# PecanProject/sipnet

Measured on AMD Instinct MI355X. Metric: ensemble-site-timesteps/sec, higher is better.
Workload: dtype f64; 1 GPU; c10k: 1 site(s) x 10240 members per GPU x 17520 half-hourly steps, perturbed params, default flags; sites_per_gpu=1, fast_math=True, gather=n/a (1 GPU), parallelism=ensemble-sharded x1, ranks_seen=1, devices_seen=1, kernel=stepCoopKernel<double, true, true, false>

## Files before the change

sipnet_amd/_lib.py:

```python
import ctypes as C
import os

_HERE = os.path.dirname(os.path.abspath(__file__))
LIB_PATH = os.path.join(_HERE, "libsipnet_amd.so")

NPARAMS, NFLAGS, NCLIM, NREC, NSTATE, RING_SLOTS = 80, 12, 11, 44, 32, 250
NDBG = 72
NREC_OUT = 36

OK = 0
ERR_BAD_PARAMETER = 3
ERR_UNKNOWN_EVENT = 4
ERR_INPUT_FILE = 5
ERR_FILE_OPEN = 6
ERR_INTERNAL = 7
ERR_BAD_CLI = 8
ERR_RESTART = 9
ERR_NO_DEVICE = 100
ERR_BAD_ARGUMENT = 101

F64, F32_MIXED = 0, 1
KERNEL_AUTO, KERNEL_ONE_WAVE, KERNEL_COOP_LDS, KERNEL_COOP_HBM, KERNEL_STRICT, KERNEL_COOP_PAIR, KERNEL_COOP_QUAD = range(7)
KERNEL_COOP_NCYCLE = 7
KERNEL_COOP_NCYCLE_PAIR = 8
# ... 170 lines not shown
    "sipnet_node_pf_check": (C.c_int, [_P, _I32P]),
    "sipnet_node_pf_ancestors": (_P, [_P, C.c_int32]),
    "sipnet_node_pf_block_len": (C.c_int64, [_P]),
    "sipnet_node_destroy": (None, [_P]),
    "sipnet_node_n_devices": (C.c_int32, [_P]),
    "sipnet_node_batch": (_P, [_P, C.c_int32]),
    "sipnet_node_run_gathering_reduced": (C.c_int, [_P, C.c_int32, C.c_int32, C.c_int32, C.c_int32, C.c_int32]),
    "sipnet_node_gathered_reduced": (_P, [_P, C.c_int32, C.c_int32, _P, _P, _P]),
    "sipnet_node_reduced_in_kernel": (C.c_int32, [_P]),
    "sipnet_node_member_range": (C.c_int, [_P, C.c_int32, _I32P, _I32P]),
    "sipnet_node_collective_library": (C.c_char_p, [_P]),
    "sipnet_comm_unique_id": (C.c_int, [_P]),
    "sipnet_comm_create": (C.c_int, [_P, C.c_int32, C.c_int32, C.c_int32, C.POINTER(_P)]),
    "sipnet_comm_all_gather": (C.c_int, [_P, _P, _P, C.c_int64, _P]),
    "sipnet_comm_world": (C.c_int32, [_P]),
    "sipnet_comm_destroy": (None, [_P]),
    "sipnet_node_set_climate": (C.c_int, [_P, C.c_int32, C.c_int32, _P, _P, _P]),
    "sipnet_node_set_events": (C.c_int, [_P, C.c_int32, C.c_int32, _P]),
    "sipnet_node_set_params": (C.c_int, [_P, C.c_int32, C.c_int32, C.c_int32, _P]),
    "sipnet_node_set_math": (C.c_int, [_P, C.c_int32]),
    "sipnet_node_set_kernel": (C.c_int, [_P, C.c_int32, C.c_int32]),
    "sipnet_node_setup": (C.c_int, [_P]),
    "sipnet_node_run": (C.c_int, [_P, C.c_int32, C.c_int32]),
    "sipnet_node_sync": (C.c_int, [_P]),
    "sipnet_node_ld": (C.c_int64, [_P]),
    "sipnet_node_planes": (_P, [_P, C.c_int32]),
    "sipnet_node_stats": (_P, [_P, C.c_int32]),
    "sipnet_node_gather_stats": (C.c_int, [_P, _P]),
    "sipnet_node_gathered_stats": (_P, [_P, C.c_int32]),
    "sipnet_node_gather_planes": (C.c_int, [_P]),
    "sipnet_node_gathered_planes": (_P, [_P, C.c_int32]),
    "sipnet_node_run_gathering": (C.c_int, [_P, C.c_int32, C.c_int32, C.c_int32]),
    "sipnet_node_n_segments": (C.c_int32, [_P]),
    "sipnet_node_gathered_segment": (_P, [_P, C.c_int32, C.c_int32, C.POINTER(C.c_int32), C.POINTER(C.c_int32)]),
    "sipnet_batch_ncol": (C.c_int64, [_P]),
    "sipnet_batch_nsteps": (C.c_int32, [_P]),
    "sipnet_batch_site_nsteps": (C.c_int32, [_P, C.c_int32]),
    "sipnet_batch_get_site_series": (C.c_int, [_P, C.c_int32, _P, _P]),
    "sipnet_batch_last_kernel_ms": (C.c_double, [_P]),
    "sipnet_batch_time_next_launch": (C.c_int, [_P]),
    "sipnet_batch_pf_arm": (C.c_int, [_P, C.c_double, C.c_double, _P]),
    "sipnet_dev_alloc": (_P, [C.c_size_t]),
    "sipnet_dev_free": (None, [_P]),
    "sipnet_dev_to_host": (C.c_int, [_P, _P, C.c_size_t, _P]),
    "sipnet_dev_to_host_2d": (C.c_int, [_P, C.c_size_t, _P, C.c_size_t, C.c_size_t, C.c_size_t, _P]),
    "sipnet_dev_to_dev_2d": (C.c_int, [_P, C.c_size_t, _P, C.c_size_t, C.c_size_t, C.c_size_t, _P]),
    "sipnet_batch_set_climate_sites": (C.c_int, [_P, C.c_int32, C.c_int32, _P, _P, _P, _P]),
    "sipnet_debug_plan_compare": (C.c_int, [_P, C.c_int32, C.c_int32, _P, _P, _P, _P, _P]),
    "sipnet_batch_run_sums": (C.c_int, [_P, C.c_int32, C.c_int32, C.c_int32, _P, _P, _P, C.c_int64, _P]),
    "sipnet_batch_sums_in_kernel": (C.c_int32, [_P]),
    "sipnet_debug_set_num_cus": (C.c_int, [_P, C.c_int32]),
    "sipnet_debug_pf_barrier": (C.c_int, [_P, C.c_int32, C.c_int32]),
    "sipnet_batch_set_device_share": (C.c_int, [_P, C.c_int32]),
    "sipnet_batch_pf_info": (C.c_int, [_P, _P, _P]),
    "sipnet_stream_sync": (C.c_int, [_P]),
    "sipnet_stream_create": (_P, [C.c_int32]),
    "sipnet_stream_destroy": (None, [_P]),
    "sipnet_io_read_clim": (C.c_int, [C.c_char_p, C.c_int32, C.POINTER(_P)]),
    "sipnet_clim_nsteps": (C.c_int32, [_P]),
    "sipnet_clim_data": (_DP, [_P]),
    "sipnet_clim_year": (_I32P, [_P]),
    "sipnet_clim_day": (_I32P, [_P]),
    "sipnet_clim_free": (None, [_P]),
    "sipnet_io_read_params": (C.c_int, [C.c_char_p, _I32P, _P, _P]),
    "sipnet_param_name": (C.c_char_p, [C.c_int32]),
    "sipnet_param_index": (C.c_int32, [C.c_char_p]),
    "sipnet_io_read_events": (C.c_int, [C.c_char_p, _I32P, _P, C.POINTER(C.POINTER(Event)), _I32P]),
    "sipnet_io_free": (None, [_P]),
    "sipnet_io_format_out_header": (C.c_int, [C.c_char_p, C.c_size_t]),
    "sipnet_io_format_out_row": (C.c_int, [C.c_char_p, C.c_size_t, C.c_int32, C.c_int32, C.c_double, _P, C.c_int64]),
    "sipnet_io_write_out": (C.c_int, [C.c_char_p, C.c_int32, C.c_int32, _P, _P, _P, _P]),
    "sipnet_io_write_debug_logs": (C.c_int, [C.c_char_p, C.c_int32, C.c_int32, _P, _P, _P, _P, _P]),
    "sipnet_io_write_events_out": (C.c_int, [C.c_char_p, C.c_int32, _I32P, _P, C.c_int32, _P, _P, _P,
                                             C.c_int32, _P, _P, _P]),
    "sipnet_io_ensemble_create": (C.c_int, [C.c_char_p, C.c_int32, C.c_int32, _P, _P, _P, _P, C.c_int32, _P, _P,
                                            C.c_int32, C.c_char_p, C.POINTER(_P)]),
    "sipnet_io_ensemble_put": (C.c_int, [_P, C.c_int32, C.c_int32, C.c_int32, C.c_int32, C.c_int32, _P, C.c_int64,
                                         C.c_int32]),
    "sipnet_io_ensemble_close": (C.c_int, [_P]),
    "sipnet_io_out_column_count": (C.c_int32, []),
    "sipnet_io_out_column_index": (C.c_int32, [C.c_char_p]),
    "sipnet_io_out_column": (C.c_int, [C.c_int32, C.POINTER(C.c_char_p), _I32P, _I32P, C.POINTER(C.c_char_p)]),
    "sipnet_io_write_ensemble_block": (C.c_int, [C.c_char_p, C.c_int32, C.c_int32, _P, _P, _P, _P, _P, _P, C.c_int64,
                                                 C.c_char_p, C.c_int32, C.c_char_p]),
    "sipnet_io_read_restart": (C.c_int, [C.c_char_p, _P]),
    "sipnet_io_write_restart": (C.c_int, [C.c_char_p, _P]),
    "sipnet_restart_check": (C.c_int, [_P, _I32P, C.c_int32, C.c_int32, C.c_int32, C.c_double,
                                       C.c_double, _I32P]),
    "sipnet_restart_check_boundary_for_write": (C.c_int, [_P, _I32P]),
}

_lib = None
_DEV_LIBRARY = False


def use_library(path):
    global LIB_PATH, _DEV_LIBRARY
    if _lib is not None:
        raise RuntimeError("sipnet_amd: the library is already loaded")
    LIB_PATH = os.path.abspath(path)
    _DEV_LIBRARY = True


def lib():
    global _lib
    if _lib is None:
        if not os.path.exists(LIB_PATH):
            raise ImportError(
                f"{LIB_PATH} is missing: the HIP extension has not been built. "
                "Run `python -c 'import __graft_entry__ as g; g.build()'`. "
                "sipnet_amd has no CPU fallback.")
        try:
            import torch
        except Exception:
            pass
        _lib = C.CDLL(LIB_PATH)
        for name, (res, args) in SIGNATURES.items():
            if _DEV_LIBRARY and not hasattr(_lib, name):
                continue
            fn = getattr(_lib, name)
            fn.restype = res
            fn.argtypes = args
    return _lib


def _strip_comments(text):
    out, i, n = [], 0, len(text)
    while i < n:
        c = text[i]
        if c in "\"'":
            j = i + 1
            while j < n and text[j] != c:
                j += 2 if text[j] == "\\" else 1
            out.append(text[i:j + 1])
            i = j + 1
        elif text.startswith("//", i):
            j = text.find("\n", i)
            i = n if j < 0 else j
        elif text.startswith("/*", i):
            j = text.find("*/", i + 2)
            i = n if j < 0 else j + 2
            out.append(" ")
        else:
            out.append(c)
            i += 1
    return " ".join("".join(out).split())


def kernel_source_sha16():
    import hashlib
    h = hashlib.sha256()
    csrc = os.path.join(_HERE, "csrc")
    for name in ("step_kernel.hip", "step_fast.hip", "fast_body.inc", "step_coop.hip", "coop_mailboxes.inc", "coop_stats.inc", "coop_wave_carbon.inc",
                 "coop_wave_factor.inc", "coop_wave_light.inc", "coop_wave_soil.inc", "coop_wave_water.inc", "step_kernel.h",
                 "fast_math.h", "coop_probes.h", "plan.h"):
        h.update(name.encode())
        h.update(_strip_comments(open(os.path.join(csrc, name), "r", errors="replace").read()).encode())
    return h.hexdigest()[:16]


class SipnetError(RuntimeError):
    def __init__(self, code, where=""):
        self.code = code
        msg = lib().sipnet_last_error().decode(errors="replace")
        super().__init__(f"{where}: status {code}: {msg}")


def check(code, where=""):
    if code != OK:
        raise SipnetError(code, where)
```

sipnet_amd/csrc/step_coop.hip:

```cpp
#include <hip/hip_runtime.h>

#include <cstdio>
#include <type_traits>

#include "fast_math.h"
#include "step_kernel.h"

namespace sipnet {
#ifdef SIPNET_COOP_BOUNDED
namespace bounded {
#endif
#ifdef SIPNET_COOP_SUMS_TU
namespace sums2 {
#endif
namespace {

constexpr int kTileBytes = kFastTile * (int)sizeof(FastRec);

#ifdef SIPNET_COOP_BOUNDED
__device__ unsigned long long g_coopStuck[2];
__shared__ int g_coopPoison;
constexpr int kSpinBudget = 1 << 22;
__device__ __forceinline__ bool spinOut(int& n, int id, int step) {
  n++;
  if ((n & 255) != 1) return false;
  int p;
  asm volatile("ds_read_b32 %0, %1\n\ts_waitcnt lgkmcnt(0)" : "=v"(p) : "v"((unsigned)(size_t)&g_coopPoison) : "memory");
  if (__builtin_amdgcn_readfirstlane(p)) return true;
  if (n < kSpinBudget) return false;
  if ((threadIdx.x & 63) == 0) {
    const unsigned long long rep = (1ull << 63) | ((unsigned long long)(unsigned)id << 32) | (unsigned)step;
    if (atomicCAS(&g_coopStuck[0], 0ull, rep) == 0ull) g_coopStuck[1] = blockIdx.x;
  }
  asm volatile("ds_write_b32 %0, %1" :: "v"((unsigned)(size_t)&g_coopPoison), "v"(1) : "memory");
  return true;
}
#define WAIT_DO for (int spin_ = 0, once_ = 1; once_; once_ = 0) do
#define WAIT_WHILE(cond, id, step) while ((cond) && !spinOut(spin_, id, step))
#else
#define WAIT_DO do
#define WAIT_WHILE(cond, id, step) while (cond)
#endif

__device__ __forceinline__ void post(double* slot, int* flag, double v, int step) {
  asm volatile("ds_write_b64 %0, %1\n\tds_write_b32 %2, %3"
               :: "v"((unsigned)(size_t)slot), "v"(v), "v"((unsigned)(size_t)flag), "v"(step) : "memory");
}
__device__ __forceinline__ void post(float* slot, int* flag, float v, int step) {
  asm volatile("ds_write_b32 %0, %1\n\tds_write_b32 %2, %3"
               :: "v"((unsigned)(size_t)slot), "v"(v), "v"((unsigned)(size_t)flag), "v"(step) : "memory");
}
__device__ __forceinline__ double take(const double* slot, const int* flag, int step) {
  double v;
  int f;
  WAIT_DO {
    asm volatile("ds_read_b32 %0, %2\n\tds_read_b64 %1, %3\n\ts_waitcnt lgkmcnt(0)"
                 : "=&v"(f), "=&v"(v) : "v"((unsigned)(size_t)flag), "v"((unsigned)(size_t)slot) : "memory");
  } WAIT_WHILE(uni(f) < step, 1, step);
  return v;
}
__device__ __forceinline__ float take(const float* slot, const int* flag, int step) {
  float v;
  int f;
  WAIT_DO {
    asm volatile("ds_read_b32 %0, %2\n\tds_read_b32 %1, %3\n\ts_waitcnt lgkmcnt(0)"
                 : "=&v"(f), "=&v"(v) : "v"((unsigned)(size_t)flag), "v"((unsigned)(size_t)slot) : "memory");
  } WAIT_WHILE(uni(f) < step, 2, step);
  return v;
}
typedef double d2_t __attribute__((ext_vector_type(2)));
typedef int i4_t __attribute__((ext_vector_type(4)));
__device__ __forceinline__ unsigned ldsAddr(const void* p) { return (unsigned)(size_t)p; }
template <class R>
__device__ __forceinline__ R q10Arg(R t10, R lg) {
  R x = t10 * lg;
  asm volatile("" : "+v"(x));
  return x;
}
__device__ __forceinline__ int aliveWord(int step, bool died) { return died ? -(step + 2) : (step + 2); }
__device__ __forceinline__ void postAlive(int* slot, int step, bool died) {
  asm volatile("ds_write_b32 %0, %1" :: "v"((unsigned)(size_t)slot), "v"(aliveWord(step, died)) : "memory");
}
__device__ __forceinline__ void takePgp(const double* slot, const int* flag, const int* alive, int step,
                                        double& pgp, bool& died) {
  int f, w;
  WAIT_DO {
    asm volatile("ds_read_b32 %0, %3\n\tds_read_b64 %1, %4\n\tds_read_b32 %2, %5\n\ts_waitcnt lgkmcnt(0)"
                 : "=&v"(f), "=&v"(pgp), "=&v"(w)
                 : "v"((unsigned)(size_t)flag), "v"((unsigned)(size_t)slot), "v"((unsigned)(size_t)alive) : "memory");
  } WAIT_WHILE(uni(f) < step || uni(w < 0 ? -w : w) < step + 2, 3, step);
  died = w < 0;
}
__device__ __forceinline__ void takePgp(const float* slot, const int* flag, const int* alive, int step,
                                        float& pgp, bool& died) {
  int f, w;
  WAIT_DO {
    asm volatile("ds_read_b32 %0, %3\n\tds_read_b32 %1, %4\n\tds_read_b32 %2, %5\n\ts_waitcnt lgkmcnt(0)"
                 : "=&v"(f), "=&v"(pgp), "=&v"(w)
                 : "v"((unsigned)(size_t)flag), "v"((unsigned)(size_t)slot), "v"((unsigned)(size_t)alive) : "memory");
  } WAIT_WHILE(uni(f) < step || uni(w < 0 ? -w : w) < step + 2, 4, step);
  died = w < 0;
}
typedef double d2v __attribute__((ext_vector_type(2)));
typedef float f2v __attribute__((ext_vector_type(2)));
typedef int i2v __attribute__((ext_vector_type(2)));
__device__ __forceinline__ void takeFactors(const double* block, const int* flags2, int step, double& g1,
                                            double& g2, double& qSoilT, double& gFine, double& gCoarse,
                                            double& moist) {
  i2v f;
  d2v a, b, c;
  WAIT_DO {
    asm volatile("ds_read2_b32 %0, %4 offset1:1\n\tds_read2st64_b64 %1, %5 offset1:1\n\t"
                 "ds_read2st64_b64 %2, %5 offset0:2 offset1:3\n\tds_read2st64_b64 %3, %5 offset0:4 offset1:5\n\t"
                 "s_waitcnt lgkmcnt(0)"
                 : "=&v"(f), "=&v"(a), "=&v"(b), "=&v"(c)
                 : "v"((unsigned)(size_t)flags2), "v"((unsigned)(size_t)block) : "memory");
  } WAIT_WHILE(uni(f.x < f.y ? f.x : f.y) < step, 5, step);
  g1 = a.x; g2 = a.y; qSoilT = b.x; gFine = b.y; gCoarse = c.x; moist = c.y;
}
__device__ __forceinline__ void takeFactors(const float* block, const int* flags2, int step, float& g1,
                                            float& g2, float& qSoilT, float& gFine, float& gCoarse, float& moist) {
  i2v f;
  f2v a, b, c;
  WAIT_DO {
    asm volatile("ds_read2_b32 %0, %4 offset1:1\n\tds_read2st64_b32 %1, %5 offset1:1\n\t"
                 "ds_read2st64_b32 %2, %5 offset0:2 offset1:3\n\tds_read2st64_b32 %3, %5 offset0:4 offset1:5\n\t"
                 "s_waitcnt lgkmcnt(0)"
                 : "=&v"(f), "=&v"(a), "=&v"(b), "=&v"(c)
                 : "v"((unsigned)(size_t)flags2), "v"((unsigned)(size_t)block) : "memory");
  } WAIT_WHILE(uni(f.x < f.y ? f.x : f.y) < step, 6, step);
  g1 = a.x; g2 = a.y; qSoilT = b.x; gFine = b.y; gCoarse = c.x; moist = c.y;
}
__device__ __forceinline__ void takeFactorsN(const double* block, const int* facFlag, const double* minNSlot, const int* minNFlag,
                                             int step, double& g1, double& g2, double& gFine, double& gCoarse, double& qSoil,
                                             double& minN, int& minNSeq) {
  int f0, f1;
  d2v a, b;
  WAIT_DO {
    asm volatile("ds_read_b32 %0, %6\n\tds_read2st64_b64 %1, %7 offset1:1\n\tds_read2st64_b64 %2, %7 offset0:3 offset1:4\n\t"
                 "ds_read_b64 %3, %7 offset:3072\n\tds_read_b32 %4, %8\n\tds_read_b64 %5, %9\n\ts_waitcnt lgkmcnt(0)"
                 : "=&v"(f0), "=&v"(a), "=&v"(b), "=&v"(qSoil), "=&v"(f1), "=&v"(minN)
                 : "v"((unsigned)(size_t)facFlag), "v"((unsigned)(size_t)block), "v"((unsigned)(size_t)minNFlag),
                   "v"((unsigned)(size_t)minNSlot) : "memory");
  } WAIT_WHILE(uni(f0) < step, 7, step);
  minNSeq = uni(f1);
  g1 = a.x; g2 = a.y; gFine = b.x; gCoarse = b.y;
}
__device__ __forceinline__ void takeFactorsN(const float* block, const int* facFlag, const double* minNSlot, const int* minNFlag,
                                             int step, float& g1, float& g2, float& gFine, float& gCoarse, float& qSoil,
                                             double& minN, int& minNSeq) {
  int f0, f1;
  f2v a, b;
  WAIT_DO {
    asm volatile("ds_read_b32 %0, %6\n\tds_read2st64_b32 %1, %7 offset1:1\n\tds_read2st64_b32 %2, %7 offset0:3 offset1:4\n\t"
                 "ds_read_b32 %3, %7 offset:1536\n\tds_read_b32 %4, %8\n\tds_read_b64 %5, %9\n\ts_waitcnt lgkmcnt(0)"
                 : "=&v"(f0), "=&v"(a), "=&v"(b), "=&v"(qSoil), "=&v"(f1), "=&v"(minN)
                 : "v"((unsigned)(size_t)facFlag), "v"((unsigned)(size_t)block), "v"((unsigned)(size_t)minNFlag),
                   "v"((unsigned)(size_t)minNSlot) : "memory");
  } WAIT_WHILE(uni(f0) < step, 8, step);
  minNSeq = uni(f1);
  g1 = a.x; g2 = a.y; gFine = b.x; gCoarse = b.y;
}
__device__ __forceinline__ void takeFactorsRing(const double* block, const int* flags2, unsigned ringAddr,
                                                int step, double& g1, double& g2, double& qSoilT,
                                                double& gFine, double& gCoarse, double& moist, double& ringV) {
  i2v f;
  d2v a, b, c;
  WAIT_DO {
    asm volatile("ds_read2_b32 %0, %5 offset1:1\n\tds_read2st64_b64 %1, %6 offset1:1\n\t"
                 "ds_read2st64_b64 %2, %6 offset0:2 offset1:3\n\tds_read2st64_b64 %3, %6 offset0:4 offset1:5\n\t"
                 "ds_read_b64 %4, %7\n\ts_waitcnt lgkmcnt(0)"
                 : "=&v"(f), "=&v"(a), "=&v"(b), "=&v"(c), "=&v"(ringV)
                 : "v"((unsigned)(size_t)flags2), "v"((unsigned)(size_t)block), "v"(ringAddr) : "memory");
  } WAIT_WHILE(uni(f.x < f.y ? f.x : f.y) < step, 9, step);
  g1 = a.x; g2 = a.y; qSoilT = b.x; gFine = b.y; gCoarse = c.x; moist = c.y;
}
__device__ __forceinline__ void takeFactorsRing(const float* block, const int* flags2, unsigned ringAddr,
                                                int step, float& g1, float& g2, float& qSoilT, float& gFine,
                                                float& gCoarse, float& moist, double& ringV) {
  i2v f;
  f2v a, b, c;
  WAIT_DO {
    asm volatile("ds_read2_b32 %0, %5 offset1:1\n\tds_read2st64_b32 %1, %6 offset1:1\n\t"
                 "ds_read2st64_b32 %2, %6 offset0:2 offset1:3\n\tds_read2st64_b32 %3, %6 offset0:4 offset1:5\n\t"
                 "ds_read_b64 %4, %7\n\ts_waitcnt lgkmcnt(0)"
                 : "=&v"(f), "=&v"(a), "=&v"(b), "=&v"(c), "=&v"(ringV)
                 : "v"((unsigned)(size_t)flags2), "v"((unsigned)(size_t)block), "v"(ringAddr) : "memory");
  } WAIT_WHILE(uni(f.x < f.y ? f.x : f.y) < step, 10, step);
  g1 = a.x; g2 = a.y; qSoilT = b.x; gFine = b.y; gCoarse = c.x; moist = c.y;
}
__device__ __forceinline__ void post5(double* base, int* flag, double v0, double v1, double v2, double v3,
                                      double v4, int step) {
  asm volatile("ds_write2st64_b64 %0, %1, %2 offset1:1\n\tds_write2st64_b64 %0, %3, %4 offset0:2 offset1:3\n\t"
               "ds_write_b64 %0, %5 offset:2048\n\tds_write_b32 %6, %7"
               :: "v"(ldsAddr(base)), "v"(v0), "v"(v1), "v"(v2), "v"(v3), "v"(v4), "v"(ldsAddr(flag)), "v"(step)
               : "memory");
}
__device__ __forceinline__ void post5(float* base, int* flag, float v0, float v1, float v2, float v3,
                                      float v4, int step) {
  asm volatile("ds_write2st64_b32 %0, %1, %2 offset1:1\n\tds_write2st64_b32 %0, %3, %4 offset0:2 offset1:3\n\t"
               "ds_write_b32 %0, %5 offset:1024\n\tds_write_b32 %6, %7"
               :: "v"(ldsAddr(base)), "v"(v0), "v"(v1), "v"(v2), "v"(v3), "v"(v4), "v"(ldsAddr(flag)), "v"(step)
               : "memory");
}
__device__ __forceinline__ void post2(double* base, int* flag, double v0, double v1, int step) {
  asm volatile("ds_write2st64_b64 %0, %1, %2 offset1:1\n\tds_write_b32 %3, %4"
               :: "v"(ldsAddr(base)), "v"(v0), "v"(v1), "v"(ldsAddr(flag)), "v"(step) : "memory");
}
__device__ __forceinline__ void post2(float* base, int* flag, float v0, float v1, int step) {
  asm volatile("ds_write2st64_b32 %0, %1, %2 offset1:1\n\tds_write_b32 %3, %4"
               :: "v"(ldsAddr(base)), "v"(v0), "v"(v1), "v"(ldsAddr(flag)), "v"(step) : "memory");
}
__device__ __forceinline__ void takeFactors7(const double* block, const int* flags2, int step, double& g1, double& g2,
                                             double& qSoilT, double& gFine, double& gCoarse, double& moist, double& mK) {
  i2v f;
  d2v a, b, c;
  WAIT_DO {
    asm volatile("ds_read2_b32 %0, %5 offset1:1\n\tds_read2st64_b64 %1, %6 offset1:1\n\t"
                 "ds_read2st64_b64 %2, %6 offset0:2 offset1:3\n\tds_read2st64_b64 %3, %6 offset0:4 offset1:5\n\t"
                 "ds_read_b64 %4, %6 offset:3072\n\ts_waitcnt lgkmcnt(0)"
                 : "=&v"(f), "=&v"(a), "=&v"(b), "=&v"(c), "=&v"(mK)
                 : "v"((unsigned)(size_t)flags2), "v"((unsigned)(size_t)block) : "memory");
  } WAIT_WHILE(uni(f.x < f.y ? f.x : f.y) < step, 11, step);
  g1 = a.x; g2 = a.y; qSoilT = b.x; gFine = b.y; gCoarse = c.x; moist = c.y;
}
__device__ __forceinline__ void takeFactors7(const float* block, const int* flags2, int step, float& g1, float& g2,
                                             float& qSoilT, float& gFine, float& gCoarse, float& moist, float& mK) {
  i2v f;
  f2v a, b, c;
  WAIT_DO {
    asm volatile("ds_read2_b32 %0, %5 offset1:1\n\tds_read2st64_b32 %1, %6 offset1:1\n\t"
                 "ds_read2st64_b32 %2, %6 offset0:2 offset1:3\n\tds_read2st64_b32 %3, %6 offset0:4 offset1:5\n\t"
                 "ds_read_b32 %4, %6 offset:1536\n\ts_waitcnt lgkmcnt(0)"
                 : "=&v"(f), "=&v"(a), "=&v"(b), "=&v"(c), "=&v"(mK)
                 : "v"((unsigned)(size_t)flags2), "v"((unsigned)(size_t)block) : "memory");
  } WAIT_WHILE(uni(f.x < f.y ? f.x : f.y) < step, 12, step);
  g1 = a.x; g2 = a.y; qSoilT = b.x; gFine = b.y; gCoarse = c.x; moist = c.y;
}
__device__ __forceinline__ void takeFactorsRing7(const double* block, const int* flags2, unsigned ringAddr, int step,
                                                 double& g1, double& g2, double& qSoilT, double& gFine, double& gCoarse,
                                                 double& moist, double& mK, double& ringV) {
  i2v f;
  d2v a, b, c;
  WAIT_DO {
    asm volatile("ds_read2_b32 %0, %6 offset1:1\n\tds_read2st64_b64 %1, %7 offset1:1\n\t"
                 "ds_read2st64_b64 %2, %7 offset0:2 offset1:3\n\tds_read2st64_b64 %3, %7 offset0:4 offset1:5\n\t"
                 "ds_read_b64 %4, %7 offset:3072\n\tds_read_b64 %5, %8\n\ts_waitcnt lgkmcnt(0)"
                 : "=&v"(f), "=&v"(a), "=&v"(b), "=&v"(c), "=&v"(mK), "=&v"(ringV)
                 : "v"((unsigned)(size_t)flags2), "v"((unsigned)(size_t)block), "v"(ringAddr) : "memory");
  } WAIT_WHILE(uni(f.x < f.y ? f.x : f.y) < step, 13, step);
  g1 = a.x; g2 = a.y; qSoilT = b.x; gFine = b.y; gCoarse = c.x; moist = c.y;
}
__device__ __forceinline__ void takeFactorsRing7(const float* block, const int* flags2, unsigned ringAddr, int step,
                                                 float& g1, float& g2, float& qSoilT, float& gFine, float& gCoarse,
                                                 float& moist, float& mK, double& ringV) {
  i2v f;
  f2v a, b, c;
  WAIT_DO {
    asm volatile("ds_read2_b32 %0, %6 offset1:1\n\tds_read2st64_b32 %1, %7 offset1:1\n\t"
                 "ds_read2st64_b32 %2, %7 offset0:2 offset1:3\n\tds_read2st64_b32 %3, %7 offset0:4 offset1:5\n\t"
                 "ds_read_b32 %4, %7 offset:1536\n\tds_read_b64 %5, %8\n\ts_waitcnt lgkmcnt(0)"
                 : "=&v"(f), "=&v"(a), "=&v"(b), "=&v"(c), "=&v"(mK), "=&v"(ringV)
                 : "v"((unsigned)(size_t)flags2), "v"((unsigned)(size_t)block), "v"(ringAddr) : "memory");
  } WAIT_WHILE(uni(f.x < f.y ? f.x : f.y) < step, 14, step);
  g1 = a.x; g2 = a.y; qSoilT = b.x; gFine = b.y; gCoarse = c.x; moist = c.y;
}
__device__ __forceinline__ void postRaw(double* p, double v) {
  asm volatile("ds_write_b64 %0, %1" :: "v"((unsigned)(size_t)p), "v"(v) : "memory");
}
__device__ __forceinline__ void postRaw(float* p, float v) {
  asm volatile("ds_write_b32 %0, %1" :: "v"((unsigned)(size_t)p), "v"(v) : "memory");
}
__device__ __forceinline__ void takeR2(const double* a, const double* b, const int* flag, int step, double& va, double& vb) {
  int f;
  WAIT_DO {
    asm volatile("ds_read_b32 %0, %3\n\tds_read_b64 %1, %4\n\tds_read_b64 %2, %5\n\ts_waitcnt lgkmcnt(0)"
                 : "=&v"(f), "=&v"(va), "=&v"(vb)
                 : "v"((unsigned)(size_t)flag), "v"((unsigned)(size_t)a), "v"((unsigned)(size_t)b) : "memory");
  } WAIT_WHILE(uni(f) < step, 15, step);
}
__device__ __forceinline__ void takeR2(const float* a, const float* b, const int* flag, int step, float& va, float& vb) {
  int f;
  WAIT_DO {
    asm volatile("ds_read_b32 %0, %3\n\tds_read_b32 %1, %4\n\tds_read_b32 %2, %5\n\ts_waitcnt lgkmcnt(0)"
                 : "=&v"(f), "=&v"(va), "=&v"(vb)
                 : "v"((unsigned)(size_t)flag), "v"((unsigned)(size_t)a), "v"((unsigned)(size_t)b) : "memory");
  } WAIT_WHILE(uni(f) < step, 16, step);
}
__device__ __forceinline__ void postD(double* row0, int k, double v) {
  asm volatile("ds_write_b64 %0, %1" :: "v"((unsigned)(size_t)(row0 + 64 * k)), "v"(v) : "memory");
}
__device__ __forceinline__ void postFlag(int* flag, int step) {
  asm volatile("ds_write_b32 %0, %1" :: "v"((unsigned)(size_t)flag), "v"(step) : "memory");
}
__device__ __forceinline__ void takeD1(const double* b, const int* flag, int step, double& v0) {
  int f;
  WAIT_DO {
    asm volatile("ds_read_b32 %0, %2\n\tds_read_b64 %1, %3\n\ts_waitcnt lgkmcnt(0)"
                 : "=&v"(f), "=&v"(v0) : "v"((unsigned)(size_t)flag), "v"((unsigned)(size_t)b) : "memory");
  } WAIT_WHILE(uni(f) < step, 17, step);
}
__device__ __forceinline__ void takeD3(const double* b, const int* flag, int step, double& v0, double& v1, double& v2) {
  int f;
  WAIT_DO {
    asm volatile("ds_read_b32 %0, %4\n\tds_read_b64 %1, %5\n\tds_read_b64 %2, %5 offset:512\n\t"
                 "ds_read_b64 %3, %5 offset:1024\n\ts_waitcnt lgkmcnt(0)"
                 : "=&v"(f), "=&v"(v0), "=&v"(v1), "=&v"(v2)
                 : "v"((unsigned)(size_t)flag), "v"((unsigned)(size_t)b) : "memory");
  } WAIT_WHILE(uni(f) < step, 18, step);
}
__device__ __forceinline__ void takeD4(const double* b, const int* flag, int step, double& v0, double& v1, double& v2,
                                       double& v3) {
  int f;
  WAIT_DO {
    asm volatile("ds_read_b32 %0, %5\n\tds_read_b64 %1, %6\n\tds_read_b64 %2, %6 offset:512\n\t"
                 "ds_read_b64 %3, %6 offset:1024\n\tds_read_b64 %4, %6 offset:1536\n\ts_waitcnt lgkmcnt(0)"
                 : "=&v"(f), "=&v"(v0), "=&v"(v1), "=&v"(v2), "=&v"(v3)
                 : "v"((unsigned)(size_t)flag), "v"((unsigned)(size_t)b) : "memory");
  } WAIT_WHILE(uni(f) < step, 19, step);
}
__device__ __forceinline__ void takeD6(const double* b, const int* flag, int step, double& v0, double& v1, double& v2,
                                       double& v3, double& v4, double& v5) {
  int f;
  WAIT_DO {
    asm volatile("ds_read_b32 %0, %7\n\tds_read_b64 %1, %8\n\tds_read_b64 %2, %8 offset:512\n\t"
                 "ds_read_b64 %3, %8 offset:1024\n\tds_read_b64 %4, %8 offset:1536\n\t"
                 "ds_read_b64 %5, %8 offset:2048\n\tds_read_b64 %6, %8 offset:2560\n\ts_waitcnt lgkmcnt(0)"
                 : "=&v"(f), "=&v"(v0), "=&v"(v1), "=&v"(v2), "=&v"(v3), "=&v"(v4), "=&v"(v5)
                 : "v"((unsigned)(size_t)flag), "v"((unsigned)(size_t)b) : "memory");
  } WAIT_WHILE(uni(f) < step, 20, step);
}
__device__ __forceinline__ void takeD8(const double* b, const int* flag, int step, double& v0, double& v1, double& v2,
                                       double& v3, double& v4, double& v5, double& v6, double& v7) {
  int f;
  WAIT_DO {
    asm volatile("ds_read_b32 %0, %9\n\tds_read_b64 %1, %10\n\tds_read_b64 %2, %10 offset:512\n\t"
                 "ds_read_b64 %3, %10 offset:1024\n\tds_read_b64 %4, %10 offset:1536\n\t"
                 "ds_read_b64 %5, %10 offset:2048\n\tds_read_b64 %6, %10 offset:2560\n\t"
                 "ds_read_b64 %7, %10 offset:3072\n\tds_read_b64 %8, %10 offset:3584\n\ts_waitcnt lgkmcnt(0)"
                 : "=&v"(f), "=&v"(v0), "=&v"(v1), "=&v"(v2), "=&v"(v3), "=&v"(v4), "=&v"(v5), "=&v"(v6), "=&v"(v7)
                 : "v"((unsigned)(size_t)flag), "v"((unsigned)(size_t)b) : "memory");
  } WAIT_WHILE(uni(f) < step, 21, step);
}
__device__ __forceinline__ bool nPlentiful(double minN, double qSoil, double len, double nVolFrac, double nLeachFrac,
                                           double demand) {
#pragma clang fp contract(off)
  const double lossShare = (nVolFrac * qSoil + nLeachFrac) * len;
  const double lower = minN * (1.0 - lossShare);
  return !(demand * len > lower);
}
__device__ __forceinline__ void awaitAtLeast(const int* flag, int step) {
  int f;
  WAIT_DO {
    asm volatile("ds_read_b32 %0, %1\n\ts_waitcnt lgkmcnt(0)" : "=v"(f) : "v"((unsigned)(size_t)flag) : "memory");
  } WAIT_WHILE(uni(f) < step, 22, step);
}

__device__ __forceinline__ void accum(double& pool, double x, double len) { pool = __builtin_fma(x, len, pool); }
__device__ __forceinline__ void accum(double& pool, float x, float len) { pool += (double)(x * len); }

#include "coop_probes.h"
}

template <class R, bool PlainExp, bool RingLds, bool Full, int NP, bool NCyc, bool Ext, bool Sums = false>
__device__ constexpr int coopCodePhase(int role) {
#ifdef SIPNET_PH_C
  if (role == 0) return SIPNET_PH_C;
#endif
#ifdef SIPNET_PH_W
  if (role == 1) return SIPNET_PH_W;
#endif
#ifdef SIPNET_PH_L
  if (role == 2) return SIPNET_PH_L;
#endif
#ifdef SIPNET_PH_F
  if (role == 3) return SIPNET_PH_F;
#endif
  if (Sums && sizeof(R) == 8 && NP == 1 && RingLds && !NCyc && !Ext && (role == 0 || role == 1)) return 3;
  if (role == 0) {
    if (NCyc) return 0;
    if (Ext) return 7;
    if (NP == 2) return 2;
    if (NP == 1 && RingLds) return Full ? 4 : 6;
    return 0;
  }
  if (role == 1) {
    if (NCyc) return 0;
    if (Ext) return 1;
    if (NP == 2) return 4;
    if (NP == 1 && RingLds) return Full ? 5 : 6;
    return 0;
  }
  if (role == 2) return (NP == 1 && RingLds && !Full && !NCyc && !Ext) ? 3 : 0;
  if (role == 3) return (NCyc && NP == 1) ? 4 : 0;
  if (role != 4) return 0;
#ifdef SIPNET_PAD_NOPS
  return SIPNET_PAD_NOPS;
#else
  constexpr bool f64 = sizeof(R) == 8;
  if (NCyc) return 4;
  if (Ext) return 4;
  if (NP == 4) return f64 ? 6 : 3;
  if (NP == 2) return Full ? 0 : f64 ? 4 : 7;
  if (!RingLds) return 0;
  return (Full || f64) ? 3 : 4;
#endif
}

template <bool On>
struct CoopSums {
  double nee = 0.0, et = 0.0, gpp = 0.0;
  int left = 0;
};
template <>
struct CoopSums<false> {};
template <class R, bool PlainExp, bool RingLds, bool Full, int NP, bool NCyc = false, bool Ext = false, bool Sums = false, bool PairDiag = false>
__device__ __forceinline__ void coopBody(const FastArgs& a) {
  static_assert(!PairDiag || (NCyc && Full && NP == 2), "PairDiag: the nitrogen cycle's two-chunk full-state layout");
  static_assert(!Sums || !Full, "in-kernel sums: lean launches");
  using OutT = typename std::conditional<Sums, double, R>::type;
  static_assert(!(NP > 1 && RingLds), "two chunks' rings do not fit one CU's LDS");
  static_assert(!NCyc || (NP <= 2 && !RingLds), "nitrogen-cycle layout: one or two chunks, ring in HBM");
  constexpr bool Opt = Ext && !NCyc;
  const bool F_growthResp = Ext && a.flags[SIPNET_F_GROWTH_RESP] != 0, F_leafWater = Ext && a.flags[SIPNET_F_LEAF_WATER] != 0;
  const bool F_flooding = Ext && a.flags[SIPNET_F_FLOODING] != 0, F_carbonSat = Ext && a.flags[SIPNET_F_CARBON_SATURATION] != 0;
  const bool F_litterPool = Opt && a.flags[SIPNET_F_LITTER_POOL] != 0, F_anaerobic = Opt && a.flags[SIPNET_F_ANAEROBIC] != 0;
  constexpr double kNoCap = 3.0e38;
  constexpr bool Pair = NP == 2;
  constexpr bool FacWave = RingLds || (Pair && !NCyc);
#include "coop_mailboxes.inc"
#ifdef SIPNET_NO_STATS
  const bool stageOn = false;
#else
  const bool stageOn = Staged && a.statsPart != nullptr;
#endif
  [[maybe_unused]] const bool firstChunk = blockIdx.x == 0 && sub == 0;
  PROBE_HWID(blockIdx.x * NP + sub, role)
  unsigned char* lds = ldsTilesAll[sub][(role < 0 || role > (NCyc ? 3 : 2)) ? 0 : role];

  const int chunksPerSite = (a.n_members + 63) >> 6;
  int site, chunk;
  {
    const int pb = (int)blockIdx.x;
    if ((a.n_sites & 7) == 0) {
      const int g = pb & 7, j = (pb >> 3) * NP + sub;
      site = g + 8 * (j / chunksPerSite);
      chunk = j % chunksPerSite;
    } else {
      const int b = pb * NP + sub;
      site = b / chunksPerSite;
      chunk = b % chunksPerSite;
    }
  }
  bool present = uni((int)(site < a.n_sites)) != 0 && role >= 0;
  if (!present) site = 0, chunk = 0;
  int m = (chunk << 6) + lane;
  const bool live = m < a.n_members;
  if (!live) m = a.n_members - 1;
  const int64_t col = (int64_t)site * a.n_members + m;
  const int opBase = uni(a.siteBase[3 * site]), evBase = uni(a.siteBase[3 * site + 1]);
  const int64_t nc = a.ncol;
  double* __restrict__ stp = a.state + col;
  const bool skip = stp[(int64_t)ST_status * nc] != 0.0;
  const bool act = live && !skip;
  const double* __restrict__ pp = a.prm + col;
#define PRM(name) (pp[(int64_t)SP_##name * nc])
#define PRM_RARE(name) ((R)pp[(int64_t)SP_##name * nc])
#define ST(name) stp[(int64_t)ST_##name * nc]

  const int siteSteps = uni(a.siteBase[3 * site + 2]);
  const int tBegin = a.step0, tEnd = a.step0 + a.n_steps < siteSteps ? a.step0 + a.n_steps : siteSteps;
  present = present && tBegin < tEnd;
#define COOP_CODE_PHASE(ROLE) \
  asm volatile("s_nop %1\n .p2align 5\n .rept %0\n s_nop 0\n .endr" ::"n"(coopCodePhase<R, PlainExp, RingLds, Full, NP, NCyc, Ext, Sums>(ROLE)), "n"(8 + (ROLE)))
  COOP_CODE_PHASE(4);
  if (role == 0) {
    if (lane == 0) {
      seqLai = tBegin - 1;
      seqPgp = tBegin - 1;
      seqPsn = tBegin - 1;
      seqFac = tBegin - 1;
      seqMoist = tBegin - 1;
      seqDone[0] = 0;
      seqDone[1] = 0;
      if (NCyc) {
        seqPlant = tBegin - 1;
        seqMinN = tBegin - 1;
        seqStorN = tBegin - 1;
        seqEvent = tBegin - 1;
        seqSupply = tBegin - 1;
        seqDemand = tBegin - 1;
        seqWat = tBegin - 1;
        seqLeach = tBegin - 1;
      }
    }
    mailAlive[0][lane] = 0;
    mailAlive[1][lane] = 0;
  }
#ifdef SIPNET_COOP_BOUNDED
  if (threadIdx.x == 0) g_coopPoison = 0;
#endif
  __syncthreads();
  if (!present) return;

  const unsigned char* __restrict__ planBytes =
      (const unsigned char*)(a.fast + (int64_t)site * a.n_steps_total);
  const Exp2Coef EC = loadExp2Coef();

#include "coop_stats.inc"
#include "coop_wave_factor.inc"
  auto tileFirst = [&](int tile) -> int64_t {
    int64_t first = (int64_t)tile * kFastTile;
    const int64_t lastStart = (int64_t)a.n_steps_total - kFastTile;
    if (first > lastStart) first = lastStart > 0 ? lastStart : 0;
    return first;
  };
  auto stageTile = [&](int tile, int buf) {
    const unsigned char* src = planBytes + tileFirst(tile) * (int64_t)sizeof(FastRec);
#pragma unroll
    for (int k = 0; k < kTileBytes / 1024; k++) {
      __builtin_amdgcn_global_load_lds(
          (const __attribute__((address_space(1))) void*)(src + k * 1024 + lane * 16),
          (__attribute__((address_space(3))) void*)(lds + buf * kTileBytes + k * 1024), 16, 0, 0);
    }
  };
  typedef double d2 __attribute__((ext_vector_type(2)));
  typedef int i4 __attribute__((ext_vector_type(4)));
  int curTile = tBegin / kFastTile;
  stageTile(curTile, curTile & 1);
  __builtin_amdgcn_s_waitcnt(0);

#include "coop_wave_soil.inc"

#include "coop_wave_light.inc"

#include "coop_wave_water.inc"

#include "coop_wave_carbon.inc"
#undef ST
#undef PRM
#undef PRM_RARE
#undef seqFac
#undef seqMoist
}

template <class R, bool PlainExp, bool RingLds, bool Full>
__global__ __launch_bounds__(RingLds ? 256 : 192) void stepCoopKernel(FastArgs a) {
  coopBody<R, PlainExp, RingLds, Full, 1>(a);
}

template <class R, bool PlainExp, bool Full>
__global__ __launch_bounds__(512) void stepCoopPairKernel(FastArgs a) {
  coopBody<R, PlainExp, false, Full, 2>(a);
}

template <class R, bool PlainExp>
__global__ __launch_bounds__(768) void stepCoopQuadKernel(FastArgs a) {
  coopBody<R, PlainExp, false, false, 4>(a);
}
#ifndef SIPNET_COOP_BOUNDED
template <bool PlainExp, bool RingLds>
__global__ __launch_bounds__(RingLds ? 256 : 192) void stepCoopSumsKernel(FastArgs a) {
  coopBody<double, PlainExp, RingLds, false, 1, false, false, true>(a);
}
template <bool PlainExp>
__global__ __launch_bounds__(512) void stepCoopPairSumsKernel(FastArgs a) {
  coopBody<double, PlainExp, false, false, 2, false, false, true>(a);
}
template <bool PlainExp, bool RingLds>
__global__ __launch_bounds__(RingLds ? 256 : 192) void stepCoopXSumsKernel(FastArgs a) {
  coopBody<double, PlainExp, RingLds, false, 1, false, true, true>(a);
}
template <bool PlainExp>
__global__ __launch_bounds__(512) void stepCoopXPairSumsKernel(FastArgs a) {
  coopBody<double, PlainExp, false, false, 2, false, true, true>(a);
}
template <bool PlainExp, bool Ext>
__global__ __launch_bounds__(256) void stepCoopNSumsKernel(FastArgs a) {
  coopBody<double, PlainExp, false, false, 1, true, Ext, true>(a);
}
template <bool PlainExp, bool Ext>
__global__ __launch_bounds__(512) void stepCoopNPairSumsKernel(FastArgs a) {
  coopBody<double, PlainExp, false, false, 2, true, Ext, true>(a);
}
#endif


template <class R, bool PlainExp>
__global__ __launch_bounds__(256) void stepCoopNKernel(FastArgs a) {
  coopBody<R, PlainExp, false, false, 1, true>(a);
}
template <class R, bool PlainExp>
__global__ __launch_bounds__(512) void stepCoopNPairKernel(FastArgs a) {
  coopBody<R, PlainExp, false, false, 2, true>(a);
}

template <class R, bool PlainExp>
__global__ __launch_bounds__(256) void stepCoopNFullKernel(FastArgs a) {
  coopBody<R, PlainExp, false, true, 1, true>(a);
}
template <class R, bool PlainExp>
__global__ __launch_bounds__(512) void stepCoopNPairFullKernel(FastArgs a) {
  coopBody<R, PlainExp, false, true, 2, true>(a);
}
#ifndef SIPNET_COOP_BOUNDED
template <class R, bool PlainExp>
__global__ __launch_bounds__(512) void stepCoopNPairDiagKernel(FastArgs a) {
  coopBody<R, PlainExp, false, true, 2, true, false, false, true>(a);
}
#endif

template <class R, bool PlainExp, bool RingLds, bool Full>
__global__ __launch_bounds__(RingLds ? 256 : 192) void stepCoopXKernel(FastArgs a) {
  coopBody<R, PlainExp, RingLds, Full, 1, false, true>(a);
}
template <class R, bool PlainExp, bool Full>
__global__ __launch_bounds__(512) void stepCoopXPairKernel(FastArgs a) {
  coopBody<R, PlainExp, false, Full, 2, false, true>(a);
}
template <class R, bool PlainExp>
__global__ __launch_bounds__(768) void stepCoopXQuadKernel(FastArgs a) {
  coopBody<R, PlainExp, false, false, 4, false, true>(a);
}
#if defined(SIPNET_PROBES) && defined(SIPNET_PROBE_XQUAD_F64)
template __global__ void stepCoopXQuadKernel<double, true>(FastArgs);
#endif
template <class R, bool PlainExp>
__global__ __launch_bounds__(256) void stepCoopNXKernel(FastArgs a) {
  coopBody<R, PlainExp, false, false, 1, true, true>(a);
}
template <class R, bool PlainExp>
__global__ __launch_bounds__(512) void stepCoopNXPairKernel(FastArgs a) {
  coopBody<R, PlainExp, false, false, 2, true, true>(a);
}
template <class R, bool PlainExp>
__global__ __launch_bounds__(256) void stepCoopNXFullKernel(FastArgs a) {
  coopBody<R, PlainExp, false, true, 1, true, true>(a);
}
template <class R, bool PlainExp>
__global__ __launch_bounds__(512) void stepCoopNXPairFullKernel(FastArgs a) {
  coopBody<R, PlainExp, false, true, 2, true, true>(a);
}
#ifndef SIPNET_COOP_BOUNDED
template <class R, bool PlainExp>
__global__ __launch_bounds__(512) void stepCoopNXPairDiagKernel(FastArgs a) {
  coopBody<R, PlainExp, false, true, 2, true, true, false, true>(a);
}
#endif

#ifdef SIPNET_COOP_SUMS_TU
template <class R, bool PlainExp, int Layout, bool Ext>
__global__ __launch_bounds__(Layout == COOP_RING_LDS ? 256 : Layout == COOP_RING_HBM ? 192 : Layout == COOP_QUAD ? 768
                             : Layout == COOP_NCYCLE ? 256 : 512) void stepCoopSumsAtKernel(FastArgs a) {
  constexpr bool N = Layout == COOP_NCYCLE || Layout == COOP_NCYCLE_PAIR;
  constexpr int NP = (Layout == COOP_PAIR || Layout == COOP_NCYCLE_PAIR) ? 2 : Layout == COOP_QUAD ? 4 : 1;
  coopBody<R, PlainExp, Layout == COOP_RING_LDS, false, NP, N, Ext, true>(a);
}
#endif

#if defined(SIPNET_HWID) && !defined(SIPNET_COOP_SUMS_TU)
extern "C" int sipnet_debug_read_coop_hwid(unsigned* out) {
  return (int)hipMemcpyFromSymbol(out, HIP_SYMBOL(g_coopHwId), sizeof(unsigned) * 4096 * 4 * 2);
}
#endif
#if defined(SIPNET_WAITS) && !defined(SIPNET_COOP_SUMS_TU)
extern "C" int sipnet_debug_read_coop_waits(unsigned long long* out) {
  return (int)hipMemcpyFromSymbol(out, HIP_SYMBOL(g_coopWaits), 16 * sizeof(unsigned long long));
}
#endif
#if defined(SIPNET_STAMPS) && !defined(SIPNET_COOP_SUMS_TU)
extern "C" int sipnet_debug_read_coop_stamps(unsigned long long* out) {
  return (int)hipMemcpyFromSymbol(out, HIP_SYMBOL(g_coopStamps), 8 * sizeof(unsigned long long));
}
#endif

#ifdef SIPNET_COOP_BOUNDED
int readCoopStuck(unsigned long long out[2], hipStream_t stream) {
  if (hipStreamSynchronize(stream) != hipSuccess) return 1;
  return (int)hipMemcpyFromSymbol(out, HIP_SYMBOL(g_coopStuck), 2 * sizeof(unsigned long long));
}
#endif
#ifdef SIPNET_COOP_SUMS_TU
void launchStepCoopSums(const FastArgs& a, int precision, int layout, hipStream_t stream, LaunchInfo* info) {
  const int chunksPerSite = (a.n_members + 63) / 64, chunks = a.n_sites * chunksPerSite;
  const bool nFamily = layout == COOP_NCYCLE || layout == COOP_NCYCLE_PAIR;
  const bool ext = nFamily ? !isNCycleFlagSet(a.flags) : !isDefaultFlagSet(a.flags);
  const bool x8 = (a.n_sites & 7) == 0;
  const int per = (layout == COOP_PAIR || layout == COOP_NCYCLE_PAIR) ? 2 : layout == COOP_QUAD ? 4 : 1;
  const int groups = per == 1 ? chunks : x8 ? 8 * ((chunks / 8 + per - 1) / per) : (chunks + per - 1) / per;
  const int threads = layout == COOP_RING_LDS ? 256 : layout == COOP_RING_HBM ? 192 : layout == COOP_QUAD ? 768 : layout == COOP_NCYCLE ? 256 : 512;
  const dim3 grid(groups), block(threads);
// ... 219 lines not shown
```

Measured before the change: 21.45 billion ensemble-site-timesteps/s.

## Add trimmed fp64 water wave for the lean single-chunk LDS-ring coop kernel

Adds a specialized water-wave body for the lean, default-physics, fp64, single-chunk LDS-ring configuration. It batches record and flag reads into one inline-asm LDS sequence, posts mailbox values through a raw ds_write helper, and uses precomputed addresses and strides held in SGPRs. It also checks the LAI sequence against a value prefetched in that batch before spinning. The aim is to shorten the water wave's per-step critical path and the handshake latency between waves. In exchange it duplicates physics logic, adds hand-tuned nop padding for code alignment, and depends on the exact record layout offsets.

```diff
diff --git a/sipnet_amd/_lib.py b/sipnet_amd/_lib.py
--- a/sipnet_amd/_lib.py
+++ b/sipnet_amd/_lib.py
@@ -346,7 +346,7 @@
     h = hashlib.sha256()
     csrc = os.path.join(_HERE, "csrc")
     for name in ("step_kernel.hip", "step_fast.hip", "fast_body.inc", "step_coop.hip", "coop_mailboxes.inc", "coop_stats.inc", "coop_wave_carbon.inc",
-                 "coop_wave_factor.inc", "coop_wave_light.inc", "coop_wave_soil.inc", "coop_wave_water.inc", "step_kernel.h",
+                 "coop_wave_factor.inc", "coop_wave_light.inc", "coop_wave_soil.inc", "coop_wave_water.inc", "coop_wave_water_trim.inc", "step_kernel.h",
                  "fast_math.h", "coop_probes.h", "plan.h"):
         h.update(name.encode())
         h.update(_strip_comments(open(os.path.join(csrc, name), "r", errors="replace").read()).encode())
diff --git a/sipnet_amd/csrc/coop_wave_water_trim.inc b/sipnet_amd/csrc/coop_wave_water_trim.inc
--- /dev/null
+++ b/sipnet_amd/csrc/coop_wave_water_trim.inc
@@ -0,0 +1,195 @@
+
+  if (role == 1) {
+    static_assert(sizeof(R) == 8 && !NCyc && !Ext && !Full && RingLds && NP == 1, "the trimmed water wave: one chunk, LDS ring, lean, default physics, fp64");
+    COOP_CODE_PHASE(1);
+    const R K_tr = (R)(1000.0 * (44.0 / 12.0) * (1.0 / 10000.0) / PRM(wueConst));
+    const R K_whc = (R)PRM(soilWHC), K_invWhc = (R)(1.0 / PRM(soilWHC));
+    const R K_wrf = (R)PRM(waterRemoveFrac);
+    const R K_frozThr = (R)PRM(frozenSoilThreshold), K_frozEff = (R)PRM(frozenSoilEff);
+    const R K_immed = (R)PRM(immedEvapFrac), K_ff = (R)PRM(fastFlowFrac);
+    const R K_invRd = (R)(1.0 / PRM(rdConst)), K_rd = (R)PRM(rdConst), K_melt = (R)PRM(snowMelt);
+    const R K_c1l = (R)(PRM(rSoilConst1) * kLog2e), K_c2l = (R)(PRM(rSoilConst2) * kLog2e);
+    const R K_moistExp = (R)PRM(soilRespMoistEffect);
+    double soilWater = ST(soilWater), snow = ST(snow);
+    double totGpp = ST(totGpp);
+    OutT* __restrict__ oEt = (OutT*)(a.et ? a.et : a.scratchRow) + col;
+    OutT* __restrict__ oGpp = (OutT*)(a.gpp ? a.gpp : a.scratchRow) + col;
+    const int64_t ldEt = a.et ? a.ld : 0, ldGpp = a.gpp ? a.ld : 0;
+    CoopSums<Sums> sumsW;
+    if constexpr (Sums) sumsW.left = a.sumEvery;
+    WAIT_DECL()
+    unsigned wRecA = 0, wMoistA = ldsAddr(&mailFac[tBegin & 1][5][lane]);
+    int wSeqV = 0;
+    unsigned wRecStride;
+    asm("s_movk_i32 %0, %1" : "=s"(wRecStride) : "n"((int)sizeof(FastRec)));
+    COOP_TRIM_PAD(10);
+    const unsigned wMoistX = ldsAddr(&mailFac[0][5][lane]) ^ ldsAddr(&mailFac[1][5][lane]);
+
+    for (int tileStart = curTile * kFastTile; tileStart < tEnd; tileStart += kFastTile, curTile++) {
+      if constexpr (Sums) {
+        if (tileStart > tBegin) asm volatile("s_waitcnt vmcnt(0)" ::: "memory");
+      } else {
+        if (tileStart > tBegin) asm volatile("s_waitcnt vmcnt(2)" ::: "memory");
+      }
+      stageTile(curTile + 1, (curTile + 1) & 1);
+      const int tFirst = tileStart > tBegin ? tileStart : tBegin;
+      const int tLast = (tileStart + kFastTile) < tEnd ? (tileStart + kFastTile) : tEnd;
+      const unsigned char* recB = lds + (curTile & 1) * kTileBytes +
+                                  (int)(tFirst - tileFirst(curTile)) * (int)sizeof(FastRec);
+      asm("v_mov_b32 %0, %2\n\tv_mov_b32 %1, %3" : "=&v"(wRecA), "=&v"(wSeqV) : "s"(ldsAddr(recB)), "s"(tFirst));
+      COOP_TRIM_PAD(5);
+      for (int t = tFirst; t < tLast; t++) {
+#pragma clang fp contract(off)
+        MARK("W step begin")
+        d2 q0, q1, q2, q3, q4, q5;
+        i2v bitsEv;
+        int wLaiSeen;
+        asm volatile("ds_read_b128 %0, %8\n\tds_read_b128 %1, %8 offset:16\n\tds_read_b64 %2, %8 offset:40\n\t"
+                     "ds_read_b64 %3, %8 offset:56\n\tds_read_b128 %4, %8 offset:64\n\t"
+                     "ds_read_b64 %5, %8 offset:80\n\tds_read2_b32 %6, %8 offset0:32 offset1:35\n\t"
+                     "ds_read_b32 %7, %9\n\ts_waitcnt lgkmcnt(0)"
+                     : "=&v"(q0), "=&v"(q1), "=&v"(q2.y), "=&v"(q3.y), "=&v"(q4), "=&v"(q5.x), "=&v"(bitsEv), "=&v"(wLaiSeen)
+                     : "v"(wRecA), "v"(ldsAddr(&seqLai)) : "memory");
+        const int32_t* rareI = (const int32_t*)(recB + (t - tFirst) * (int)sizeof(FastRec) + 184);
+        const R len = (R)q0.x, invLen = (R)q0.y, tair = recR<R>(q1.x), tsoil = recR<R>(q1.y);
+        const int bits = uni(bitsEv.x);
+        const R eWater = (R)soilWater, eSnow = (R)snow;
+        const bool frozen = tsoil < K_frozThr;
+
+        {
+          R moistEff = clip01(eWater * K_invWhc);
+          if (!PlainExp && __builtin_amdgcn_ballot_w64(K_moistExp != R(1)) != 0)
+            moistEff = (K_moistExp == R(1)) ? moistEff : fpow(moistEff, K_moistExp);
+          moistEff = (bits & FAST_TSOIL_NEG) ? R(1) : moistEff;
+          postAt(wMoistA, ldsAddr(&seqMoist), moistEff, wSeqV);
+        }
+
+        const bool tairPos = (bits & FAST_TAIR_POS) != 0;
+        const R rate = recR<R>(q3.y);
+        const R rain = tairPos ? rate : R(0), snowFall = tairPos ? R(0) : rate;
+        const R netRain = ffma(-rain, K_immed, rain);
+        R snowMelt = 0, sublimation = 0, evaporationPot = 0;
+        const bool hasSnow = eSnow > R(0);
+        if (hasSnow) {
+          R subl = rmax0(recR<R>(q4.x) * K_invRd);
+          R remaining = ffma(snowFall, len, eSnow);
+          const R afterSubl = ffma(-subl, len, remaining);
+          const bool allGone = afterSubl < R(0);
+          subl = allGone ? remaining * invLen : subl;
+          remaining = allGone ? R(0) : afterSubl;
+          R melt = tairPos ? K_melt * tair : R(0);
+          melt = (tairPos && (ffma(-melt, len, remaining) < R(0))) ? remaining * invLen : melt;
+          sublimation = subl;
+          snowMelt = melt;
+        } else {
+          const R wf = clip01(eWater * K_invWhc);
+          const R rsoil = fexp2(ffma(-K_c2l, wf, K_c1l), EC);
+          evaporationPot = rmax0(fdiv(recR<R>(q4.y), ffma(K_rd, recR<R>(q5.x), rsoil)));
+        }
+        R removable = rminv(eWater, K_whc) * K_wrf;
+        removable = frozen ? removable * K_frozEff : removable;
+
+        R transpiration = 0, photosynthesis = 0;
+        if (bits & FAST_PAR_POS) {
+          R pgpSpec;
+          bool diedBefore;
+          WAIT_BEGIN()
+          unsigned wSlotOff = (unsigned)(((t & 1) * 64 + lane) * (int)sizeof(R));
+          asm("" : "+v"(wSlotOff));
+          takePgp((const R*)(size_t)(ldsAddr(&mailPgp[0][0]) + wSlotOff), &seqPgp, &mailAlive[t & 1][lane], t, pgpSpec, diedBefore);
+          WAIT_END(0)
+          const R potGrossPsn = diedBefore ? R(0) : pgpSpec;
+          const R potTrans = potGrossPsn * recR<R>(q2.y) * K_tr;
+          const bool hasPsn = potGrossPsn >= R(kTiny);
+          const bool limited = hasPsn && removable < potTrans;
+          transpiration = hasPsn ? (limited ? removable : potTrans) : R(0);
+          photosynthesis = potGrossPsn;
+          if (__builtin_expect(__builtin_amdgcn_ballot_w64(limited) != 0, 0))
+            photosynthesis = limited ? potGrossPsn * fdiv(removable, potTrans) : potGrossPsn;
+          postAt(ldsAddr(&mailPsn[0][0]) + wSlotOff, ldsAddr(&seqPsn), photosynthesis, wSeqV);
+        }
+        wMoistA ^= wMoistX;
+        wSeqV += 1;
+        wRecA += wRecStride;
+        const R tGpp = photosynthesis * len;
+        totGpp += (double)tGpp;
+
+        R evaporation, drainage, wetting;
+        {
+          R netIn = netRain + snowMelt;
+          wetting = ffma(-netIn, K_ff, ffma(-rain, K_immed, rain + snowMelt));
+          netIn = ffma(-netIn, K_ff, netIn);
+          R remaining = ffma(-transpiration, len, ffma(netIn, len, eWater));
+          const R afterEvap = ffma(-evaporationPot, len, remaining);
+          const bool dryOut = !hasSnow && (afterEvap < R(kTiny));
+          evaporation = dryOut ? (remaining - R(kTiny)) * invLen : evaporationPot;
+          remaining = hasSnow ? remaining : (dryOut ? R(0) : afterEvap);
+          drainage = remaining > K_whc ? (remaining - K_whc) * invLen : R(0);
+        }
+        R evEvap = 0;
+        if (__builtin_expect(__builtin_amdgcn_ballot_w64(bitsEv.y > 0) != 0, 0)) {
+          R evSoilWater = 0;
+          const int ev0 = uni(rareI[3]);
+          const int nEv = uni(bitsEv.y);
+          COOP_TRIM_PAD(3);
+          for (int k = 0; k < nEv; k++) {
+            const EvRec& ev = a.events[evBase + ev0 + k];
+            if (uni(ev.type) == SIPNET_EV_IRRIG) {
+              const R p0 = (R)ev.p[0];
+              const R evapAmount = ((int)ev.p[1] == 0) ? K_immed * p0 : R(0);
+              evEvap = ffma(evapAmount, invLen, evEvap);
+              evSoilWater = ffma(p0 - evapAmount, invLen, evSoilWater);
+            }
+          }
+          accum(soilWater, evSoilWater, len);
+        }
+        accum(soilWater, wetting - evaporation - transpiration - drainage, len);
+        accum(snow, snowFall - snowMelt - sublimation, len);
+        soilWater = rmax0(soilWater);
+        snow = snow < kTiny ? 0.0 : snow;
+
+        if (!(bits & FAST_PAR_POS)) {
+          WAIT_BEGIN()
+          awaitAtLeastSeen(&seqLai, t, wLaiSeen);
+          WAIT_END(1)
+        }
+
+        const R tEt = (ffma(rain, K_immed, transpiration) + evaporation + sublimation + evEvap) * len;
+        if constexpr (Sums) {
+          sumsW.et += (double)tEt;
+          sumsW.gpp += (double)tGpp;
+          if (--sumsW.left == 0) {
+            *oEt = (OutT)sumsW.et;
+            *oGpp = (OutT)sumsW.gpp;
+            oEt += ldEt;
+            oGpp += ldGpp;
+            sumsW.et = sumsW.gpp = 0.0;
+            sumsW.left = a.sumEvery;
+          }
+        } else {
+          *oEt = tEt;
+          *oGpp = tGpp;
+          oEt += ldEt;
+          oGpp += ldGpp;
+        }
+        MARK("W step end")
+      }
+    }
+    if constexpr (Sums) {
+      if (sumsW.left != a.sumEvery) {
+        *oEt = (OutT)sumsW.et;
+        *oGpp = (OutT)sumsW.gpp;
+      }
+    }
+    WAIT_STORE(4)
+    if (a.statsPart) {
+      asm volatile("s_waitcnt vmcnt(0)" ::: "memory");
+      asm volatile("ds_write_b32 %0, %1" :: "v"(ldsAddr(&seqDone[1])), "v"(1) : "memory");
+    }
+    if (act) {
+      ST(soilWater) = soilWater;
+      ST(snow) = snow;
+      ST(totGpp) = totGpp;
+    }
+    return;
+  }
diff --git a/sipnet_amd/csrc/step_coop.hip b/sipnet_amd/csrc/step_coop.hip
--- a/sipnet_amd/csrc/step_coop.hip
+++ b/sipnet_amd/csrc/step_coop.hip
@@ -101,6 +101,9 @@
   } WAIT_WHILE(uni(f) < step || uni(w < 0 ? -w : w) < step + 2, 4, step);
   died = w < 0;
 }
+__device__ __forceinline__ void postAt(unsigned slot, unsigned flag, double v, int stepV) {
+  asm volatile("ds_write_b64 %0, %1\n\tds_write_b32 %2, %3" :: "v"(slot), "v"(v), "v"(flag), "v"(stepV) : "memory");
+}
 typedef double d2v __attribute__((ext_vector_type(2)));
 typedef float f2v __attribute__((ext_vector_type(2)));
 typedef int i2v __attribute__((ext_vector_type(2)));
@@ -354,6 +357,16 @@
   WAIT_DO {
     asm volatile("ds_read_b32 %0, %1\n\ts_waitcnt lgkmcnt(0)" : "=v"(f) : "v"((unsigned)(size_t)flag) : "memory");
   } WAIT_WHILE(uni(f) < step, 22, step);
+}
+__device__ __forceinline__ void awaitAtLeastSeen(const int* flag, int step, int seen) {
+#ifdef SIPNET_COOP_BOUNDED
+  if (uni(seen) < step) awaitAtLeast(flag, step);
+#else
+  int f;
+  asm volatile("1:\n\tv_readfirstlane_b32 %1, %0\n\ts_cmp_ge_i32 %1, %3\n\ts_cbranch_scc1 2f\n\t"
+               "ds_read_b32 %0, %2\n\ts_waitcnt lgkmcnt(0)\n\ts_branch 1b\n2:"
+               : "+v"(seen), "=&s"(f) : "v"((unsigned)(size_t)flag), "s"(step) : "memory", "scc");
+#endif
 }
 
 __device__ __forceinline__ void accum(double& pool, double x, double len) { pool = __builtin_fma(x, len, pool); }
@@ -429,6 +442,7 @@
   constexpr bool Pair = NP == 2;
   constexpr bool FacWave = RingLds || (Pair && !NCyc);
 #include "coop_mailboxes.inc"
+  constexpr bool Trim = NP == 1 && RingLds && !Full && !NCyc && !Ext && sizeof(R) == 8;
 #ifdef SIPNET_NO_STATS
   const bool stageOn = false;
 #else
@@ -473,6 +487,7 @@
   present = present && tBegin < tEnd;
 #define COOP_CODE_PHASE(ROLE) \
   asm volatile("s_nop %1\n .p2align 5\n .rept %0\n s_nop 0\n .endr" ::"n"(coopCodePhase<R, PlainExp, RingLds, Full, NP, NCyc, Ext, Sums>(ROLE)), "n"(8 + (ROLE)))
+#define COOP_TRIM_PAD(N) asm volatile(".rept %0\n s_nop 0\n .endr" ::"n"(N))
   COOP_CODE_PHASE(4);
   if (role == 0) {
     if (lane == 0) {
@@ -534,9 +549,14 @@
 
 #include "coop_wave_light.inc"
 
+  if constexpr (Trim) {
+#include "coop_wave_water_trim.inc"
+  } else {
 #include "coop_wave_water.inc"
+  }
 
 #include "coop_wave_carbon.inc"
+#undef COOP_TRIM_PAD
 #undef ST
 #undef PRM
 #undef PRM_RARE
```

Result: no change. 21.58 billion ensemble-site-timesteps/s, median of 6 (+0.6%).
